# ilyamaclean/microclimf

Hardware: AMD Instinct MI355X
Metric: cell-steps/s (higher is better)
Workload: dtype f64

## Files before the change

microclimf_amd/csrc/mcf_device.hpp:

```cpp
#pragma once
#include <hip/hip_runtime.h>
#include <stdint.h>

#include "mcf_kernels.h"


namespace mcf {

constexpr double kPi = 3.14159265358979323846;
constexpr double kToRad = kPi / 180.0;
constexpr double kSb = 5.67e-8;
constexpr double kThetam = 0.365;
constexpr double kKa = 0.4;
constexpr double kOmdy = (2.0 * kPi) / (24.0 * 3600.0);
constexpr uint64_t kNaRealBits = 0x7FF00000000007A2ULL;

enum : int {
    FL_VALID = 1,
    FL_PAI = 2,
    FL_BELOW = 4,
    FL_XONE = 8,
    FL_XINF = 16,
    FL_XZERO = 32,
    FL_ABOVE1 = 64,
// ... 318 lines not shown
            if (vconst) asm volatile("" : "+s"(t[4]));
            if (vconst) asm volatile("" : "+v"(c5));
            if (vconst || lean_fast) {
                asm volatile("" : "+v"(magic));
                asm volatile("" : "+v"(sh3));
                vfast = true;
            }
        } else {
#pragma unroll
            for (int i = 0; i < 12; ++i) asm volatile("" : "+s"(e[i]));
        }
        if (with_log) {
#pragma unroll
            for (int i = 0; i < 7; ++i)
                if (!logtab) asm volatile("" : "+s"(l[i]));
                else if (i > 0) asm volatile("" : "+s"(g[i]));
            if (logtab && vconst) asm volatile("" : "+v"(g7v));
        }
        if (!vconst) return;
        if (!table) asm volatile("" : "+v"(c11));
        if (with_log && !logtab) { asm volatile("" : "+v"(lg6)); asm volatile("" : "+v"(lg7)); }
    }
};
template <bool BOUNDED, bool SHORT = false>
__device__ __forceinline__ double fexp_tab(double x, const MathK& K) {
    double n, r, p, r2, out;
    int t;
    if (BOUNDED && K.vfast) {
        double y;
        asm("v_fma_f64 %0, %1, %2, %3" : "=v"(y) : "v"(x), "s"(K.t[0]), "v"(K.magic));
        t = __double2loint(y);
        asm("v_add_f64 %0, %1, -%2" : "=v"(n) : "v"(y), "v"(K.magic));
    } else {
        asm("v_mul_f64 %0, %1, %2\n\t"
            "v_rndne_f64 %0, %0"
            : "=v"(n) : "v"(x), "s"(K.t[0]));
        asm("v_cvt_i32_f64 %0, %1" : "=v"(t) : "v"(n));
    }
    if (BOUNDED && SHORT && K.vfast) {
        asm("v_fma_f64 %0, %1, %2, %3" : "=v"(r) : "v"(n), "s"(K.t[4]), "v"(x));
    } else {
        asm("v_fma_f64 %0, %1, %2, %3\n\t"
            "v_fma_f64 %0, %1, %4, %0"
            : "=&v"(r) : "v"(n), "s"(K.t[1]), "v"(x), "s"(K.t[2]));
    }
    double T;
    if (K.vfast) {
        unsigned off;
        asm("v_lshlrev_b32_sdwa %0, %1, %2 dst_sel:DWORD dst_unused:UNUSED_PAD src0_sel:DWORD src1_sel:BYTE_0"
            : "=v"(off) : "v"(K.sh3), "v"(t));
        T = *reinterpret_cast<const double*>(reinterpret_cast<const char*>(K.tab) + off);
    } else {
        T = K.tab[t & 255];
    }
    const int e = t >> 8;
    asm("v_fma_f64 %0, %2, %3, %4\n\t"
        "v_fma_f64 %0, %2, %0, 0.5\n\t"
        "v_mul_f64 %1, %2, %2\n\t"
        "v_fma_f64 %0, %1, %0, %2"
        : "=&v"(p), "=&v"(r2)
        : "v"(r), "s"(K.t[3]), "v"(K.c5));
    asm("v_fma_f64 %0, %1, %2, %1\n\t"
        "v_ldexp_f64 %0, %0, %3"
        : "=&v"(out)
        : "v"(T), "v"(p), "v"(e));
    return out;
}
__device__ __forceinline__ double fexp(double x, const MathK& K);
template <bool F = true>
__device__ __forceinline__ double fexp_b(double x, const MathK& K) {
    if (F && K.table) return fexp_tab<true>(x, K);
    return fexp(x, K);
}
template <bool F = true>
__device__ __forceinline__ double fexp_s(double x, const MathK& K) {
    if (F && K.table) return fexp_tab<true, true>(x, K);
    return fexp(x, K);
}
__device__ __forceinline__ double fexp(double x, const MathK& K) {
    if (K.table) return fexp_tab<false>(x, K);
    double n, r, p, out;
    int t;
    const double c11 = K.c11;
    asm("v_mul_f64 %0, %5, %6\n\t"
        "v_rndne_f64 %0, %0\n\t"
        "v_fma_f64 %1, %0, %7, %5\n\t"
        "v_fma_f64 %1, %0, %8, %1\n\t"
        "v_fma_f64 %2, %1, %9, %10\n\t"
        "v_fma_f64 %2, %1, %2, %11\n\t"
        "v_fma_f64 %2, %1, %2, %12\n\t"
        "v_fma_f64 %2, %1, %2, %13\n\t"
        "v_fma_f64 %2, %1, %2, %14\n\t"
        "v_fma_f64 %2, %1, %2, %15\n\t"
        "v_fma_f64 %2, %1, %2, %16\n\t"
        "v_fma_f64 %2, %1, %2, %17\n\t"
        "v_fma_f64 %2, %1, %2, %18\n\t"
        "v_fma_f64 %2, %1, %2, 1.0\n\t"
        "v_fma_f64 %2, %1, %2, 1.0\n\t"
        "v_cvt_i32_f64 %3, %0\n\t"
        "v_ldexp_f64 %4, %2, %3"
        : "=&v"(n), "=&v"(r), "=&v"(p), "=&v"(t), "=v"(out)
        : "v"(x), "s"(K.e[0]), "s"(K.e[1]), "s"(K.e[2]), "v"(c11), "s"(K.e[3]), "s"(K.e[4]), "s"(K.e[5]), "s"(K.e[6]),
          "s"(K.e[7]), "s"(K.e[8]), "s"(K.e[9]), "s"(K.e[10]), "s"(K.e[11]));
    return out;
}
__device__ __forceinline__ double flog_tab(double x, const MathK& K) {
    const double m = __builtin_amdgcn_frexp_mant(x);
    int e = __builtin_amdgcn_frexp_exp(x);
    const int j = (__double2hiint(m) >> 12) & 255;
    const double2 cl = *reinterpret_cast<const double2*>(K.ltab + 2 * j);
    e -= j < kLogSplit ? 1 : 0;
    const double dk = (double)e;
    double r, q, r2, out;
    asm("v_fma_f64 %0, %4, %5, -1.0\n\t"
        "v_fma_f64 %1, %0, %7, %8\n\t"
        "v_fma_f64 %1, %0, %1, %9\n\t"
        "v_fma_f64 %1, %0, %1, %10\n\t"
        "v_fma_f64 %1, %0, %1, %11\n\t"
        "v_fma_f64 %1, %0, %1, -0.5\n\t"
        "v_mul_f64 %2, %0, %0\n\t"
        "v_fma_f64 %1, %2, %1, %0\n\t"
        "v_fma_f64 %1, %6, %12, %1\n\t"
        "v_fma_f64 %3, %6, %13, %14\n\t"
        "v_add_f64 %3, %3, %1"
        : "=&v"(r), "=&v"(q), "=&v"(r2), "=&v"(out)
        : "v"(m), "v"(cl.x), "v"(dk), "v"(K.g7v), "s"(K.g[1]), "s"(K.g[2]), "s"(K.g[3]), "s"(K.g[4]), "s"(K.g[5]), "s"(K.g[6]),
          "v"(cl.y));
    return out;
}
__device__ __forceinline__ double flog(double x, const MathK& K) {
    if (K.logtab) return flog_tab(x, K);
    double m = __builtin_amdgcn_frexp_mant(x);
    int e = __builtin_amdgcn_frexp_exp(x);
    const int lo = m < 0.70710678118654752440 ? 1 : 0;
    m = __builtin_amdgcn_ldexp(m, lo);
    e -= lo;
    const double f = m - 1.0;
    const double s = fdiv(f, 2.0 + f);
    const double hfsq = 0.5 * f * f;
    const double dk = (double)e;
    const double lg6 = K.lg6, lg7 = K.lg7;
    double z, w, t1, t2, out;
    asm("v_mul_f64 %0, %5, %5\n\t"
        "v_mul_f64 %1, %0, %0\n\t"
        "v_fma_f64 %2, %1, %9, %10\n\t"
        "v_fma_f64 %3, %1, %11, %12\n\t"
        "v_fma_f64 %2, %1, %2, %13\n\t"
        "v_fma_f64 %3, %1, %3, %14\n\t"
        "v_mul_f64 %2, %1, %2\n\t"
        "v_fma_f64 %3, %1, %3, %15\n\t"
        "v_fma_f64 %2, %0, %3, %2\n\t"
        "v_add_f64 %2, %6, %2\n\t"
        "v_mul_f64 %2, %5, %2\n\t"
        "v_fma_f64 %2, %8, %16, %2\n\t"
        "v_add_f64 %2, %6, -%2\n\t"
        "v_add_f64 %2, %2, -%7\n\t"
        "v_fma_f64 %4, %8, %17, -%2"
        : "=&v"(z), "=&v"(w), "=&v"(t1), "=&v"(t2), "=v"(out)
        : "v"(s), "v"(hfsq), "v"(f), "v"(dk), "v"(lg6), "s"(K.l[0]), "v"(lg7), "s"(K.l[1]), "s"(K.l[2]), "s"(K.l[3]),
          "s"(K.l[4]), "s"(K.l[5]), "s"(K.l[6]));
    return out;
}
__device__ __forceinline__ double powxy(double x, double y, const MathK& K) { return fexp(y * flog(x, K), K); }
__device__ __forceinline__ double sq(double x) { return x * x; }
__device__ __forceinline__ double pow4(double x) { double x2 = x * x; return x2 * x2; }

__device__ __forceinline__ void satvap_nd(double tc, double& num, double& den) {
    const bool water = tc > 0;
    const uint64_t m = __builtin_amdgcn_ballot_w64(water);
    if (m == __builtin_amdgcn_ballot_w64(true)) { num = 17.27 * tc; den = tc + 237.3; asm("" : "+v"(num), "+v"(den)); }
    else if (m == 0) { num = 21.875 * tc; den = tc + 265.5; asm("" : "+v"(num), "+v"(den)); }
    else { num = (water ? 17.27 : 21.875) * tc; den = tc + (water ? 237.3 : 265.5); }
}
__device__ __forceinline__ double satvap_arg(double tc) {
    double num, den;
    satvap_nd(tc, num, den);
    return fdiv(num, den);
}
__device__ __forceinline__ void frcp2(double a, double b, double& ra, double& rb) {
    const double r = frcp(a * b);
    ra = r * b;
    rb = r * a;
}
__device__ __forceinline__ void frcp2_m(double a, double b, double& ra, double& rb) {
    const double r = frcp_m(a * b);
    ra = r * b;
    rb = r * a;
}
__device__ __forceinline__ double satvap(double tc, const MathK& K) { return 0.61078 * fexp(satvap_arg(tc), K); }
constexpr double kLnSvp0 = -0x1.f8d9d41e4b1ffp-2;
template <bool F>
__device__ __forceinline__ double satvap_f(double t, const MathK& K) {
    if (F && K.table) {
        double num, den;
        satvap_nd(t, num, den);
        return fexp_s<true>(fma(num, frcp(den), kLnSvp0), K);
    }
    return 0.61078 * fexp_b<F>(satvap_arg(t), K);
}
template <bool F>
__device__ __forceinline__ double satvap_rd(double num, double rden, const MathK& K) {
    if (F && K.table) return fexp_s<true>(fma(num, rden, kLnSvp0), K);
    return 0.61078 * fexp_b<F>(num * rden, K);
}
__device__ __forceinline__ double lw_emit(double tc) { return 0.97 * kSb * pow4(tc + 273.15); }
__device__ __forceinline__ double latent(double tc) {
    return tc >= 0 ? 45068.7 - 42.8428 * tc : 51078.69 - 4.338 * tc - 0.06367 * tc * tc;
}

struct SolPos { double zend, zenr, azid; };

__host__ __device__ inline int julday(int year, int month, int day) {
    double dd = day + 0.5;
    int madj = month + (month < 3) * 12;
    int yadj = year + (month < 3) * -1;
    double j = trunc(365.25 * (yadj + 4716)) + trunc(30.6001 * (madj + 1)) + dd - 1524.5;
    int b = (int)(2 - trunc((double)(yadj / 100)) + trunc(trunc((double)(yadj / 100)) / 4));
    return (int)(j + (j > 2299160) * b);
}

struct SolDate { double sindec, cosdec, eot; };
__device__ inline SolDate sol_date(int year, int month, int day) {
    int jd = julday(year, month, day);
    double m = 6.24004077 + 0.01720197 * (jd - 2451545.0);
    SolDate s;
    s.eot = -7.659 * sin(m) + 9.863 * sin(2 * m + 3.5932);
// ... 205 lines not shown
    __device__ __forceinline__ double operator()(int field) const { return lds_operand(p, field * CPB); }
    __device__ __forceinline__ double hor(int s) const { return lds_operand(p, (CF_COUNT + s) * CPB); }
    __device__ __forceinline__ double wsa(int w) const { return lds_operand(p, (CF_COUNT + 24 + w) * CPB); }
};
struct TimeLds {
    static constexpr bool in_registers = false;
    LdsPtr row;
    __device__ __forceinline__ double operator()(int field) const { return lds_operand(row, field * 24); }
};
struct TimeReg {
    static constexpr bool in_registers = true;
    const TimeVals* t;
    __device__ __forceinline__ double operator()(int field) const { return t->v[field]; }
};

struct Carry {
    double soilm, num0, rden, radCsw, Rddown, Rbdown, X, uf;
};
struct Pass1Out {
    double Tg0, absRnet;
    double uz, Rdup;
};

__device__ __forceinline__ void pin1(double& a) { asm volatile("" : "+v"(a)); }
template <class... A>
__device__ __forceinline__ void pin(A&... a) {
    (pin1(a), ...);
}

#ifndef MCF_CANARY_ALL
#define MCF_CANARY_ALL 0
#endif
struct Canary {
    double c = 0.0;
    __device__ __forceinline__ void watch(double x) { c = fma(0.0, x, c); }
    __device__ __forceinline__ void trip() { c = __builtin_nan(""); }
    __device__ __forceinline__ bool tripped() const { return c != c; }
};
__device__ __forceinline__ void vmin64(double& x, double hi) {
    if (__builtin_constant_p(hi)) {
        if (hi == 1.0) asm("v_min_f64 %0, %0, 1.0" : "+v"(x));
        else asm("v_min_f64 %0, %0, %1" : "+v"(x) : "s"(hi));
    } else asm("v_min_f64 %0, %0, %1" : "+v"(x) : "v"(hi));
}
__device__ __forceinline__ void vmax64(double& x, double lo) {
    if (__builtin_constant_p(lo)) {
        if (lo == 0.0) asm("v_max_f64 %0, %0, 0" : "+v"(x));
        else asm("v_max_f64 %0, %0, %1" : "+v"(x) : "s"(lo));
    } else asm("v_max_f64 %0, %0, %1" : "+v"(x) : "v"(lo));
}
template <bool F>
__device__ __forceinline__ void cap(double& x, double hi, Canary& cn) {
// ... 110 lines not shown
};
struct NoDiag {
    static constexpr bool on = false;
    __device__ __forceinline__ void operator()(int, double) const {}
};
template <int NT>
struct DiagRing {
    static constexpr bool on = true;
    char* day;
    uint64_t sel;
    uint32_t posb;
    __device__ __forceinline__ void operator()(int v, double val) const {
        const unsigned s = (unsigned)(sel >> (4 * v)) & 15u;
        if (s == 15u) return;
        uint32_t pb = posb;
        asm("" : "+v"(pb));
        *(double*)(day + ((size_t)s * (NT * 8)) + pb) = val;
    }
};

template <bool F, bool SS, class CL, class TM, class SL, class DG = NoDiag>
__device__ __forceinline__ void pass1(const CL& C, const TM& T, const SL& S, const Globals& g, int flags, double dTmx,
                                      Carry& cy, Pass1Out& o, const MathK& K, Canary& cn, const DG& dg = NoDiag()) {
    double t_idx = T(TF_IDX), rsw = T(TF_RSW), rdif = T(TF_RDIF);
    pin(t_idx, rsw, rdif);
    const int idx = (int)t_idx;
    constexpr bool soil_shared = SS;
    double soilm, matric;
    if (soil_shared) {
        soilm = S(SD_SOILM);
        matric = S(SD_MATRIC);
    } else {
        double t_soilmp = T(TF_SOILMP), c_smin = C(CF_SMIN), c_invrge = C(CF_INVRGE), c_eta = C(CF_ETA), c_rge = C(CF_RGE);
        pin(t_soilmp, c_smin, c_invrge, c_eta, c_rge);
        soilm = soil_spread<F>(t_soilmp, c_smin, c_invrge, c_eta, c_rge, cn);
        matric = -C(CF_ABSPSIE) * powxy(soilm * C(CF_INVSMAX), -C(CF_SOILB), K);
    }
    cy.soilm = soilm;
    double radGsw = 0.0, radCsw = 0.0, Rbdown = 0.0, Rddown = 0.0, Rdup = 0.0, X = 0.0;
    if constexpr (DG::on) {
        if (!(rsw > 0.0)) {
            double si = T(TF_CZ) * C(CF_CS) + T(TF_SZ) * (C(CF_SSCA) * T(TF_CAZ) + C(CF_SSSA) * T(TF_SAZ));
            if (!g.shadowmask && T(TF_ZEND) > 90.0) si = 0.0;
            flr<F>(si, 0.0, cn);
            if (C.hor(idx & 31) > T(TF_TANSA)) si = 0.0;
            dg(DG_SI, si);
        }
    }
    if (rsw > 0.0) {
        double cz = T(TF_CZ), t_sz = T(TF_SZ), t_caz = T(TF_CAZ), t_saz = T(TF_SAZ), t_tansa = T(TF_TANSA),
               t_zend = T(TF_ZEND);
        double c_cs = C(CF_CS), c_ssca = C(CF_SSCA), c_sssa = C(CF_SSSA), c_hor = C.hor(idx & 31),
               svfa = C(CF_SVFA), gref = C(CF_GREF);
        pin(cz, t_sz, t_caz, t_saz, t_tansa, t_zend, c_cs, c_ssca, c_sssa, c_hor, svfa, gref);
        double si = cz * c_cs + t_sz * (c_ssca * t_caz + c_sssa * t_saz);
        if (!g.shadowmask && t_zend > 90.0) si = 0.0;
        flr<F>(si, 0.0, cn);
        if (c_hor > t_tansa) si = 0.0;
        if constexpr (DG::on) dg(DG_SI, si);
        if (flags & FL_PAI) {
            double t_tan2c = T(TF_TAN2C), t_cosc = T(TF_COSC);
            double c_xx = C(CF_XX), c_kdeninv = C(CF_KDENINV), om = C(CF_OM), gma = C(CF_GMA), agm = C(CF_AGM),
                   u1 = C(CF_U1), u2 = C(CF_U2), c_gma2 = C(CF_GMA2),
                   c_agm2 = C(CF_AGM2), c_jdel = C(CF_JDEL), c_pait = C(CF_PAIT), c_invd2 = C(CF_INVD2), c_gmagref = C(CF_GMAGREF);
            pin(t_tan2c, t_cosc, c_xx, c_kdeninv, om, gma, agm, u1, u2, c_gma2, c_agm2, c_jdel, c_pait, c_invd2, c_gmagref);
            double k = fsqrt(c_xx + t_tan2c) * c_kdeninv;
            if (flags & (FL_XONE | FL_XINF | FL_XZERO))
                k = (flags & FL_XONE) ? T(TF_INV2COSC) : (flags & FL_XINF) ? 1.0 : T(TF_TANC);
            cap<F>(k, 6000.0, cn);
            double rsi = frcp(si);
            double kd = k * t_cosc * rsi;
            double Kc = rsi;
            if (si == 0.0) { kd = 1.0; Kc = 600.0; }
            double sig = kd * kd + c_gma2 - c_agm2;
            double ss = 0.5 * (om * kd + c_jdel);
            double sstr = om * kd - ss;
            double S2 = fexp(-kd * c_pait, K);
            double isig = frcp(sig);
            double p5 = -ss * (agm - kd) - gma * sstr;
            double p5s = p5 * isig;
            double v1 = ss - (p5 * (agm + kd)) * isig;
            double v2 = ss - gma - p5s * (u1 + kd);
            double gS2v2 = S2 * v2;
            double p8 = sstr * (agm + kd) - gma * ss;
            double p8s = -p8 * isig;
            double v3 = (sstr + c_gmagref - p8s * (u2 - kd)) * S2;
            const double dv3 = c_invd2 * v3;
            double c_logclump = C(CF_LOGCLUMP), c_loggi = C(CF_LOGGI), amx = C(CF_AMX), trdn = C(CF_TRDN),
                   trdu = C(CF_TRDU), c_paiaa = C(CF_PAIAA), c_rddng = C(CF_RDDNG), c_albd = C(CF_ALBD), c_rddnz = C(CF_RDDNZ),
                   c_rdupz = C(CF_RDUPZ);
            constexpr bool late_k = TM::in_registers;
            double ka1 = late_k ? 0.0 : C(CF_KA1), ka2 = late_k ? 0.0 : C(CF_KA2), kb1 = late_k ? 0.0 : C(CF_KB1),
                   kb2 = late_k ? 0.0 : C(CF_KB2), kg1 = late_k ? 0.0 : C(CF_KG1), kg2 = late_k ? 0.0 : C(CF_KG2),
                   kz1 = late_k ? 0.0 : C(CF_KZ1), kz2 = late_k ? 0.0 : C(CF_KZ2);
            double Rbeam = T(TF_RBEAM), Rb = T(TF_RB);
            if (late_k) pin(c_logclump, c_loggi, amx, trdn, trdu, c_paiaa, c_rddng, c_albd, c_rddnz, c_rdupz, Rbeam, Rb);
            else pin(c_logclump, c_loggi, amx, trdn, trdu, c_paiaa, c_rddng, c_albd, c_rddnz, c_rdupz, ka1, ka2, kb1, kb2, kg1, kg2, kz1,
                     kz2, Rbeam, Rb);
            double trbn = fexp(Kc * c_logclump, K);
            cap<F>(trbn, 0.999, cn);
            if (!F) flr<F>(trbn, 0.0, cn);
            double trb = fexp(Kc * c_loggi, K);
            cap<F>(trb, 0.999, cn);
            if (!F) flr<F>(trb, 0.0, cn);
            if (late_k) { ka1 = C(CF_KA1); ka2 = C(CF_KA2); }
            double albb = (1.0 - trdn * trbn) * (p5s + (v1 * ka1 + gS2v2 * ka2)) + trdn * trbn * gref;
            if (F) cn.watch(albb);
            cap<F>(albb, amx, cn);
            flr<F>(albb, 0.01, cn);
            if (late_k) { kg1 = C(CF_KG1); kg2 = C(CF_KG2); }
            double Rdbdn_g = (1.0 - trbn) * (p8s * (S2 + kg1) + dv3 * kg2);
            if (F) cn.watch(Rdbdn_g);
            cap<F>(Rdbdn_g, amx, cn);
            flr<F>(Rdbdn_g, 0.0, cn);
            double S2a = fexp(-kd * c_paiaa, K);
            if (late_k) { kb1 = C(CF_KB1); kb2 = C(CF_KB2); }
            double Rdbup_z = (1.0 - trdu * trbn) * (p5s * S2a + (v1 * kb1 + gS2v2 * kb2)) + trdu * trbn * gref;
            cap<F>(Rdbup_z, amx, cn);
            flr<F>(Rdbup_z, 0.0, cn);
            if (late_k) { kz1 = C(CF_KZ1); kz2 = C(CF_KZ2); }
            double Rdbdn_z = (1.0 - trb) * (p8s * (S2a + kz1) + dv3 * kz2);
            cap<F>(Rdbdn_z, amx, cn);
            flr<F>(Rdbdn_z, 0.0, cn);
            double trg = trb + (1 - trb) * S2;
            double Rbc = (trg * si + (1 - trg) * cz) * Rbeam;
            double Rbdn_g = trbn + (1.0 - trbn) * S2;
            if (!F) {
                cap<F>(Rbdn_g, 1.0, cn);
                flr<F>(Rbdn_g, 0.0, cn);
            }
            const double rds = rdif * svfa;
            radGsw = (1.0 - gref) * (c_rddng * rds + Rdbdn_g * Rb + Rbdn_g * Rbeam * si);
            double maxg = (1.0 - gref) * (rds + Rbeam * si);
            cap<F>(radGsw, maxg, cn);
            radCsw = (1.0 - c_albd) * rds + (1.0 - albb) * Rbc;
            Rbdown = (trb + (1.0 - trb) * S2a) * Rbeam;
            Rddown = c_rddnz * rds + Rdbdn_z * Rb;
            Rdup = c_rdupz * rds + Rdbup_z * Rb;
            X = Rddown + Rdup + k * cz * Rbdown;
        } else {
            Rbdown = (rsw - rdif) / cz;
            Rddown = rdif * svfa;
            Rdup = gref * (rdif * svfa + (rsw - rdif));
            radGsw = (1.0 - gref) * (svfa * rdif + si * Rbdown);
            radCsw = radGsw;
        }
    }
    cy.radCsw = radCsw;
    cy.Rddown = Rddown;
    cy.Rbdown = Rbdown;
    cy.X = X;
    o.Rdup = Rdup;
    if constexpr (DG::on) {
        dg(DG_RADGSW, radGsw);
        dg(DG_RADCSW, radCsw);
        const bool lit = rsw > 0.0 && (flags & FL_PAI);
        dg(DG_RADLSW, lit ? C(CF_HOM) * X : 0.0);
        dg(DG_RADLPAR, lit ? C(CF_HOMP) * X : 0.0);
    }
    double c_tsv = C(CF_TSV), c_omtrdif = C(CF_OMTRDIF), ws = C.wsa((idx >> 5) & 7), c_ufc = C(CF_UFC),
           c_uzfac = C(CF_UZFAC), c_ghafac = C(CF_GHAFAC);
    double t_rlw = T(TF_RLW), t_rem = T(TF_REM), u2m = T(TF_U2), t_umu = T(TF_UMU), t_wfac = T(TF_WFAC),
           t_lapk = T(TF_LAPK), t_es = T(TF_ES), t_ea = T(TF_EA), t_ghr = T(TF_GHRRAD), t_de = T(TF_DE),
           tc = T(TF_TC), tdew = T(TF_TDEW);
    pin(c_tsv, c_omtrdif, ws, c_ufc, c_uzfac, c_ghafac, t_rlw, t_rem, u2m, t_umu,
        t_wfac, t_lapk, t_es, t_ea, t_ghr, t_de, tc, tdew);
    const double radGlw = 0.97 * (c_tsv * t_rlw + c_omtrdif * t_rem);
    if constexpr (DG::on) {
        double lwsum = c_tsv * t_rlw + c_omtrdif * t_rem;
        asm volatile("" : "+v"(lwsum));
        const double radGlw_d = 0.97 * lwsum;
        dg(DG_RADGLW, radGlw_d);
        dg(DG_RADCLW, (flags & FL_PAI) ? 0.97 * C(CF_SVFA) * t_rlw : radGlw_d);
        dg(DG_LWOUT, t_rem);
    }
    if (isnan(ws)) ws = 1.0;
    flr<F>(ws, 0.05, cn);
    double uf = u2m * c_ufc * t_umu * ws;
    flr<F>(uf, 0.001, cn);
    double uz = uf * c_uzfac;
    cap<F>(uz, u2m, cn);
    double gHa = uf * c_ghafac;
    flr<F>(gHa, 0.0001, cn);
    cy.uf = uf;
    o.uz = uz;
    if constexpr (DG::on) {
        dg(DG_UF, uf);
        dg(DG_GHA, gHa);
    }
    const double radabs = radGsw + radGlw;
    double surfwet = fexp(matric * t_wfac, K);
    if (!F) cap<F>(surfwet, 1.0, cn);
    const double m = t_lapk * gHa;
    const double num0 = radabs - t_rem - m * (t_es - t_ea) * surfwet;
    const double den = 29.3 * (gHa + t_ghr) + m * t_de;
    cy.num0 = num0;
    const double rden = frcp_m(den);
    cy.rden = rden;
    double Tg0 = pm_temperature_r<F, F && !TM::in_registers>(num0, rden, dTmx, tc, tdew, cn);
    o.Tg0 = Tg0;
    o.absRnet = fabs(radabs - lw_emit(Tg0));
}

struct Stom {
    double gsmax, rsmx, inv02rsmx, gs2;
};
template <bool F>
__device__ __forceinline__ double stomcond(double Rswabs, const Stom& s, const MathK& K, Canary& cn) {
    if (Rswabs <= 0.0) return 0.0;
    double gs = s.gsmax;
    if (Rswabs < s.rsmx) gs = s.gsmax * fexp_s<F>((Rswabs - s.rsmx) * s.inv02rsmx, K);
    cap<F>(gs, s.gs2, cn);
    return gs;
}
// ... 51 lines not shown
    flr<F>(G, -0.6 * Rmx, cn);
    const double Tg = pm_temperature_r<F, F && !TM::in_registers>(cy.num0 - G, cy.rden, dTmx, tc, tdew, cn);
    o.Tg = Tg;
    o.DD = DD;
    if constexpr (DG::on) {
        dg(DG_T0, Tg);
        dg(DG_G, G);
        dg(DG_KDDG, DD);
    }
    if (!above_ground) return;
    constexpr bool lean = TM::in_registers;
    double c_ghafac = C(CF_GHAFAC), c_smin = C(CF_SMIN), c_invrge = C(CF_INVRGE), c_pai = C(CF_PAI),
           c_ksat = C(CF_KSAT), c_psunsat = C(CF_PSUNSAT), c_shadefac = lean ? 0.0 : C(CF_SHADEFAC),
           c_ompc = lean ? 0.0 : C(CF_OMPC), c_svfa = lean ? 0.0 : C(CF_SVFA);
    double rlw = T(TF_RLW), rsw = T(TF_RSW), rdif = T(TF_RDIF), t_idx = T(TF_IDX), lapk = T(TF_LAPK),
           es = T(TF_ES), De = T(TF_DE), rem = T(TF_REM), ghr = T(TF_GHRRAD);
    if (lean) pin(c_ghafac, c_smin, c_invrge, c_pai, c_ksat, c_psunsat);
    else pin(c_ghafac, c_smin, c_invrge, c_pai, c_ksat, c_psunsat, c_shadefac, c_ompc, c_svfa, rlw, rsw, rdif, t_idx,
             lapk, es, De, rem, ghr);
    const double uf = cy.uf;
    double gHa = uf * c_ghafac;
    flr<F>(gHa, 0.0001, cn);
    constexpr bool PAIR = F && !lean;
    const double surfwet = (soilm - c_smin) * c_invrge;
    double esTg = 0.0, dgw = 0.0, gwet = 0.0;
    auto ground_wetness = [&]() {
        double eT = esTg - ea;
        flr<F>(eT, 0.001, cn);
        double plf = 0.8753 - 1.7126 * flog(eT, K);
        dgw = 1.0 + fexp_s<F>(-plf, K);
    };
    if (!PAIR) {
        esTg = satvap_f<F>(Tg, K);
        ground_wetness();
        gwet = frcp(dgw);
        flr<F>(gwet, surfwet, cn);
    }
    const int idx = (int)t_idx;
    double gS = 9999.99;
    Stom st;
    st.gs2 = 0.0;
    bool have_gs2 = false;
    auto load_stom = [&]() {
        if (soil_shared) {
            st.gsmax = C(CF_GSMAX);
            st.rsmx = C(CF_RSMX);
// ... 30 lines not shown
                inv2cosb = 1.0 / (2.0 * cos(zend));
            } else {
                tanb = T(TF_TANB); tan2b = T(TF_TAN2B); inv2cosb = T(TF_INV2COSB);
            }
            kb = fsqrt(C(CF_XX) + tan2b) * C(CF_KDENINV);
            if (flags & (FL_XONE | FL_XINF | FL_XZERO))
                kb = (flags & FL_XONE) ? inv2cosb : (flags & FL_XINF) ? 1.0 : tanb;
            cap<F>(kb, 6000.0, cn);
            P_sun = fdiv_m(1.0 - fexp(-kb * c_pai, K), kb);
        }
        double P_shade = c_pai - P_sun;
        if (lean) { c_shadefac = C(CF_SHADEFAC); c_ompc = C(CF_OMPC); }
        double Rshade_abs = rdif * c_shadefac;
        double Rsun_abs = (rsw - rdif) * kb * (1 - c_ompc) + Rshade_abs;
        double gs_sun = 0.0, gs_shade = 0.0;
        if (!(Rsun_abs <= 0.0) || !(Rshade_abs <= 0.0)) {
            load_stom();
            gs_sun = stomcond<F>(Rsun_abs, st, K, cn);
            gs_shade = stomcond<F>(Rshade_abs, st, K, cn);
        }
        gS = gs_sun * P_sun + gs_shade * P_shade;
    }
    double gV = 0.0;
    if (PAIR) {
        double nTg, dTg, rTg, rG;
        satvap_nd(Tg, nTg, dTg);
        frcp2(dTg, gHa + gS, rTg, rG);
        esTg = satvap_rd<F>(nTg, rTg, K);
        if (gS > 0.0) gV = (gHa * gS) * rG;
        ground_wetness();
    } else if (gS > 0.0) gV = fdiv_m(gHa * gS, gHa + gS);
    if (lean) c_svfa = C(CF_SVFA);
    const double Rabs = cy.radCsw + 0.97 * c_svfa * rlw;
    const double mC = lapk * gV;
    const double esw = (es - ea) * surfwet;
    const double numC = Rabs - rem - mC * esw - G, denC = 29.3 * (gHa + ghr) + mC * De;
    double Tcan;
    if (PAIR) {
        double rC;
        frcp2_m(dgw, denC, gwet, rC);
        flr<F>(gwet, surfwet, cn);
        Tcan = pm_temperature_r<F, F && !lean>(numC, rC, dTmx, tc, tdew, cn);
    } else {
        Tcan = pm_temperature<F, F && !lean>(numC, denC, dTmx, tc, tdew, cn);
    }
    double esTcan, muR = 0.0;
    if (PAIR) {
        double nTc, dTc, rTc;
        satvap_nd(Tcan, nTc, dTc);
        if (flags & FL_BELOW) frcp2(dTc, C(CF_A2H) * uf, rTc, muR);
        else rTc = frcp(dTc);
        esTcan = satvap_rd<F>(nTc, rTc, K);
    } else {
        esTcan = satvap_f<F>(Tcan, K);
    }
    midway();
    double ez;
    if (!(flags & FL_BELOW)) {
        double w = C(CF_OML1);
        bool prof = (flags & FL_ABOVE1) != 0;
        o.Tz = prof ? tc + (Tcan - tc) * w : Tcan;
        ez = prof ? ea + (esTcan - ea) * surfwet * w : ea + (esTcan - ea) * surfwet;
        o.tleaf = Tcan;
        o.lwup = lw_emit(Tcan);
        o.lwdn = rlw;
    } else {
        double c_uzfac = C(CF_UZFAC), emg = C(CF_EMG), ema = C(CF_EMA), invleafd = C(CF_INVLEAFD),
               c_hom = C(CF_HOM), c_homp = C(CF_HOMP), t_u2 = T(TF_U2);
        pin(c_uzfac, emg, ema, invleafd, c_hom, c_homp, t_u2);
        double uz = uf * c_uzfac;
        cap<F>(uz, t_u2, cn);
        const double lwcan = lw_emit(Tcan), lwgro = lw_emit(Tg);
        const double lwup = emg * lwgro + (1 - emg) * lwcan;
        const double lwdn = ema * rlw + (1 - ema) * lwcan;
        const double lwabs = 0.97 * 0.5 * (lwup + lwdn);
        const bool lit = F || (rsw > 0.0 && (flags & FL_PAI));
        const double leafabs = (lit ? c_hom * cy.X : 0.0) + lwabs;
        double gh = (0.135 * 1.4) * fsqrt_m(uz * invleafd);
        const double RnetL = leafabs - lwcan;
        bool floors_idle = false;
        {
            const double tq = gh * (1.0 / 0.0463), tq2 = tq * tq;
            const bool clear = gh >= 0.0500001 && tq2 * tq2 * tq >= (fabs(RnetL) * invleafd) * 1.000001;
            floors_idle = __builtin_amdgcn_ballot_w64(!clear) == 0;
        }
        double a02 = 0.0;
        if (!floors_idle) {
            a02 = mincond_a02<F>(RnetL, invleafd, K, cn);
            double gmin = mincond_gmin<F>(g.hf0p, a02, cn);
            flr<F>(gh, gmin, cn);
        }
        double gVl = gh;
        if (flags & FL_STOM) {
            gVl = 0.0;
            const double PARabs = lit ? c_homp * cy.X : 0.0;
            double gs = 0.0;
            if (PARabs > 0.0) {
                if (!have_gs2) load_stom();
// ... 70 lines not shown
        }
        const double HL = 29.3 * gh * (tleaf - tc);
        const double LL = mL * (esTl - ea) * surfwet;
        const double cp43 = 29.3 * 43.0;
        {
            double Flux = HC * omem, SH = Th * cp43, SG = Tg * cp43;
            double mxnear = fabs(tleaf - Th) * cp43;
            double SC = SH + Flux * rKc;
            double farg = (Kg * SG + Kh * SH + Kc * SC) * invK;
            double near = nf * (HL * lden);
            near_field_limit<F>(near, mxnear);
            o.Tz = (near + farg) * (1.0 / cp43);
        }
        {
            double Flux = LC * omem, SH = eh * mu, SG = esTg * gwet * mu;
            double mxnear = fabs(esTl - eh) * mu;
            double SC = SH + Flux * rKc;
            double farg = (Kg * SG + Kh * SH + Kc * SC) * invK;
            double near = nf * (LL * lden);
            near_field_limit<F>(near, mxnear);
            ez = (near + farg) * invmu;
        }
    }
    double rh;
    if (F) {
        rh = (ez * (100.0 / 0.61078)) * fexp_s<true>(-satvap_arg(o.Tz), K);
    } else {
        rh = fdiv(ez, satvap(o.Tz, K)) * 100.0;
    }
    if (F) cn.watch(rh);
    cap<F>(rh, 100.0, cn);
    o.rh = rh;
    double tmx = o.tleaf;
    flr<F>(tmx, tc, cn);
    flr<F>(tmx, Tg, cn);
    flr<F>(tmx, Tcan, cn);
    double tmn = o.tleaf;
    cap<F>(tmn, tc, cn);
    cap<F>(tmn, Tg, cn);
    cap<F>(tmn, Tcan, cn);
    cap<F>(o.Tz, tmx + 2.0, cn);
    flr<F>(o.Tz, tmn - 2.0, cn);
}

}
```

microclimf_amd/csrc/mcf_kernels.hip:

```cpp
#include <hip/hip_runtime.h>
#include <math.h>
#include <stdio.h>
#include <stdint.h>
#include <algorithm>

#include "mcf_device.hpp"
#include "mcf_kernels.h"

#ifndef MCF_WAVES_PER_EU
#define MCF_WAVES_PER_EU 4
#endif
#ifndef MCF_AF_WAVES
#define MCF_AF_WAVES 3
#endif

namespace mcf {

__global__ void k_fill(double* __restrict__ p, int64_t n, double v) {
    int64_t i = (int64_t)blockIdx.x * blockDim.x + threadIdx.x;
    int64_t stride = (int64_t)gridDim.x * blockDim.x;
    for (; i < n; i += stride) p[i] = v;
}

__global__ void k_gather_cells(RingView src, int64_t step0, int64_t nsteps, const int64_t* __restrict__ cells,
// ... 1634 lines not shown
    double a = x[i], b = y ? y[i] : 0.0, r;
    MathK K;
    K.set();
    __shared__ double s_exptab[256];
    K.use_table(s_exptab, (int)threadIdx.x);
    __shared__ __attribute__((aligned(16))) double s_logtab[512];
    K.use_log_table(s_logtab, (int)threadIdx.x, (int)blockDim.x);
    K.pin(true, true);
    __syncthreads();
    switch (kind) {
        case 0: r = fexp(a, K); break;
        case 1: r = flog(a, K); break;
        case 2: r = fdiv(a, b); break;
        case 3: r = fsqrt(a); break;
        case 4: r = frcp(a); break;
        case 5: r = satvap(a, K); break;
        case 7: r = fexp_b<true>(a, K); break;
        case 8: r = satvap_f<true>(a, K); break;
        case 9: r = fexp_s<true>(a, K); break;
        case 10: r = frcp_m(a); break;
        case 11: r = fsqrt_m(a); break;
        case 12: { double ra, rb; frcp2_m(a, b, ra, rb); r = ra + rb; break; }
        case 13: { double ra, rb; frcp2(a, b, ra, rb); r = ra + rb; break; }
        default: r = powxy(a, b, K); break;
    }
    if (live) out[i] = r;
}
void launch_selftest_math(int kind, const double* x, const double* y, double* out, int64_t n, hipStream_t s) {
    if (n <= 0) return;
    hipLaunchKernelGGL(k_selftest_math, dim3((unsigned)((n + 255) / 256)), dim3(256), 0, s, kind, x, y, out, n);
}

__global__ __launch_bounds__(256) void k_pack_transpose(RingView src, int64_t step0, int64_t rows, int64_t cols,
                                                        double scale, int32_t* __restrict__ dst) {
    __shared__ int32_t tile[32][33];
    const int64_t N = rows * cols;
    const int64_t step = step0 + blockIdx.z;
    int32_t* out = dst + (int64_t)blockIdx.z * N;
    const int tx = threadIdx.x & 31, ty = threadIdx.x >> 5;
    const int64_t r0 = (int64_t)blockIdx.x * 32, c0 = (int64_t)blockIdx.y * 32;
#pragma unroll
    for (int j = ty; j < 32; j += 8) {
        const int64_t r = r0 + tx, c = c0 + j;
        int32_t v = INT32_MIN;
        if (r < rows && c < cols) {
            const double x = rint(src.at(r + rows * c, step) * scale);
// ... 336 lines not shown
```

Baseline: 31.46 billion.

## Split table exp/log into issue and finish phases to hide LDS latency

Splits the LDS-table-based exp and log routines into an issue phase, which computes the index and starts the table load, and a finish phase that evaluates the polynomial. In pass1 and the canopy pass, several exp/log calls are issued early and finished later, with independent arithmetic placed in between to hide LDS load latency. Volatile LDS address-space loads plus register pins keep the compiler from sinking the loads back to their use. The cost is more live VGPRs across the overlap window, which may lower occupancy. Self-test cases for the new paths are added.

```diff
diff --git a/microclimf_amd/csrc/mcf_device.hpp b/microclimf_amd/csrc/mcf_device.hpp
--- a/microclimf_amd/csrc/mcf_device.hpp
+++ b/microclimf_amd/csrc/mcf_device.hpp
@@ -364,9 +364,20 @@
         if (with_log && !logtab) { asm volatile("" : "+v"(lg6)); asm volatile("" : "+v"(lg7)); }
     }
 };
-template <bool BOUNDED, bool SHORT = false>
-__device__ __forceinline__ double fexp_tab(double x, const MathK& K) {
-    double n, r, p, r2, out;
+__device__ __forceinline__ void pin1(double& a) { asm volatile("" : "+v"(a)); }
+template <class... A>
+__device__ __forceinline__ void pin(A&... a) {
+    (pin1(a), ...);
+}
+
+struct ExpPending {
+    double r;
+    int e;
+    double T;
+};
+template <bool BOUNDED, bool SHORT = false, bool HELD = true>
+__device__ __forceinline__ ExpPending fexp_tab_issue(double x, const MathK& K) {
+    double n, r;
     int t;
     if (BOUNDED && K.vfast) {
         double y;
@@ -386,27 +397,42 @@
             "v_fma_f64 %0, %1, %4, %0"
             : "=&v"(r) : "v"(n), "s"(K.t[1]), "v"(x), "s"(K.t[2]));
     }
-    double T;
+    typedef const volatile __attribute__((address_space(3))) char* LdsBytes;
+    typedef const volatile __attribute__((address_space(3))) double* LdsDouble;
+    ExpPending q;
     if (K.vfast) {
         unsigned off;
         asm("v_lshlrev_b32_sdwa %0, %1, %2 dst_sel:DWORD dst_unused:UNUSED_PAD src0_sel:DWORD src1_sel:BYTE_0"
             : "=v"(off) : "v"(K.sh3), "v"(t));
-        T = *reinterpret_cast<const double*>(reinterpret_cast<const char*>(K.tab) + off);
+        if (HELD) q.T = *(LdsDouble)((LdsBytes)K.tab + off);
+        else q.T = *reinterpret_cast<const double*>(reinterpret_cast<const char*>(K.tab) + off);
     } else {
-        T = K.tab[t & 255];
-    }
-    const int e = t >> 8;
+        if (HELD) q.T = ((LdsDouble)K.tab)[t & 255];
+        else q.T = K.tab[t & 255];
+    }
+    q.r = r;
+    q.e = t >> 8;
+    return q;
+}
+template <bool HELD = true>
+__device__ __forceinline__ double fexp_tab_finish(const ExpPending& q, const MathK& K) {
+    double p, r2, out, T = q.T;
     asm("v_fma_f64 %0, %2, %3, %4\n\t"
         "v_fma_f64 %0, %2, %0, 0.5\n\t"
         "v_mul_f64 %1, %2, %2\n\t"
         "v_fma_f64 %0, %1, %0, %2"
         : "=&v"(p), "=&v"(r2)
-        : "v"(r), "s"(K.t[3]), "v"(K.c5));
+        : "v"(q.r), "s"(K.t[3]), "v"(K.c5));
+    if (HELD) pin1(T);
     asm("v_fma_f64 %0, %1, %2, %1\n\t"
         "v_ldexp_f64 %0, %0, %3"
         : "=&v"(out)
-        : "v"(T), "v"(p), "v"(e));
+        : "v"(T), "v"(p), "v"(q.e));
     return out;
+}
+template <bool BOUNDED, bool SHORT = false>
+__device__ __forceinline__ double fexp_tab(double x, const MathK& K) {
+    return fexp_tab_finish<false>(fexp_tab_issue<BOUNDED, SHORT, false>(x, K), K);
 }
 __device__ __forceinline__ double fexp(double x, const MathK& K);
 template <bool F = true>
@@ -446,13 +472,35 @@
           "s"(K.e[7]), "s"(K.e[8]), "s"(K.e[9]), "s"(K.e[10]), "s"(K.e[11]));
     return out;
 }
-__device__ __forceinline__ double flog_tab(double x, const MathK& K) {
-    const double m = __builtin_amdgcn_frexp_mant(x);
-    int e = __builtin_amdgcn_frexp_exp(x);
-    const int j = (__double2hiint(m) >> 12) & 255;
-    const double2 cl = *reinterpret_cast<const double2*>(K.ltab + 2 * j);
-    e -= j < kLogSplit ? 1 : 0;
+struct LogPending {
+    double m;
+    int e, j;
+    double c, l;
+};
+template <bool HELD = true>
+__device__ __forceinline__ LogPending flog_tab_issue(double x, const MathK& K) {
+    LogPending q;
+    q.m = __builtin_amdgcn_frexp_mant(x);
+    q.e = __builtin_amdgcn_frexp_exp(x);
+    q.j = (__double2hiint(q.m) >> 12) & 255;
+    if (HELD) {
+        typedef double __attribute__((ext_vector_type(2))) LdsEntry;
+        const LdsEntry cl = *(const volatile __attribute__((address_space(3))) LdsEntry*)(K.ltab + 2 * q.j);
+        q.c = cl.x;
+        q.l = cl.y;
+    } else {
+        const double2 cl = *reinterpret_cast<const double2*>(K.ltab + 2 * q.j);
+        q.c = cl.x;
+        q.l = cl.y;
+    }
+    return q;
+}
+template <bool HELD = true>
+__device__ __forceinline__ double flog_tab_finish(const LogPending& p, const MathK& K) {
+    const int e = p.e - (p.j < kLogSplit ? 1 : 0);
     const double dk = (double)e;
+    double c = p.c, l = p.l;
+    if (HELD) pin(c, l);
     double r, q, r2, out;
     asm("v_fma_f64 %0, %4, %5, -1.0\n\t"
         "v_fma_f64 %1, %0, %7, %8\n\t"
@@ -466,10 +514,11 @@
         "v_fma_f64 %3, %6, %13, %14\n\t"
         "v_add_f64 %3, %3, %1"
         : "=&v"(r), "=&v"(q), "=&v"(r2), "=&v"(out)
-        : "v"(m), "v"(cl.x), "v"(dk), "v"(K.g7v), "s"(K.g[1]), "s"(K.g[2]), "s"(K.g[3]), "s"(K.g[4]), "s"(K.g[5]), "s"(K.g[6]),
-          "v"(cl.y));
+        : "v"(p.m), "v"(c), "v"(dk), "v"(K.g7v), "s"(K.g[1]), "s"(K.g[2]), "s"(K.g[3]), "s"(K.g[4]), "s"(K.g[5]), "s"(K.g[6]),
+          "v"(l));
     return out;
 }
+__device__ __forceinline__ double flog_tab(double x, const MathK& K) { return flog_tab_finish<false>(flog_tab_issue<false>(x, K), K); }
 __device__ __forceinline__ double flog(double x, const MathK& K) {
     if (K.logtab) return flog_tab(x, K);
     double m = __builtin_amdgcn_frexp_mant(x);
@@ -504,6 +553,42 @@
     return out;
 }
 __device__ __forceinline__ double powxy(double x, double y, const MathK& K) { return fexp(y * flog(x, K), K); }
+struct ExpLater {
+    ExpPending q = {0.0, 0, 0.0};
+    double v = 0.0;
+};
+struct LogLater {
+    LogPending q = {0.0, 0, 0, 0.0, 0.0};
+    double v = 0.0;
+};
+__device__ __forceinline__ ExpLater fexp_issue(double x, const MathK& K) {
+    ExpLater o;
+    if (K.table) o.q = fexp_tab_issue<false>(x, K);
+    else o.v = fexp(x, K);
+    return o;
+}
+template <bool F = true>
+__device__ __forceinline__ ExpLater fexp_b_issue(double x, const MathK& K) {
+    ExpLater o;
+    if (F && K.table) o.q = fexp_tab_issue<true>(x, K);
+    else o = fexp_issue(x, K);
+    return o;
+}
+template <bool F = true>
+__device__ __forceinline__ ExpLater fexp_s_issue(double x, const MathK& K) {
+    ExpLater o;
+    if (F && K.table) o.q = fexp_tab_issue<true, true>(x, K);
+    else o = fexp_issue(x, K);
+    return o;
+}
+__device__ __forceinline__ double fexp_finish(const ExpLater& o, const MathK& K) { return K.table ? fexp_tab_finish(o.q, K) : o.v; }
+__device__ __forceinline__ LogLater flog_issue(double x, const MathK& K) {
+    LogLater o;
+    if (K.logtab) o.q = flog_tab_issue(x, K);
+    else o.v = flog(x, K);
+    return o;
+}
+__device__ __forceinline__ double flog_finish(const LogLater& o, const MathK& K) { return K.logtab ? flog_tab_finish(o.q, K) : o.v; }
 __device__ __forceinline__ double sq(double x) { return x * x; }
 __device__ __forceinline__ double pow4(double x) { double x2 = x * x; return x2 * x2; }
 
@@ -544,6 +629,16 @@
 __device__ __forceinline__ double satvap_rd(double num, double rden, const MathK& K) {
     if (F && K.table) return fexp_s<true>(fma(num, rden, kLnSvp0), K);
     return 0.61078 * fexp_b<F>(num * rden, K);
+}
+template <bool F>
+__device__ __forceinline__ ExpLater satvap_rd_issue(double num, double rden, const MathK& K) {
+    if (F && K.table) return fexp_s_issue<true>(fma(num, rden, kLnSvp0), K);
+    return fexp_b_issue<F>(num * rden, K);
+}
+template <bool F>
+__device__ __forceinline__ double satvap_finish(const ExpLater& o, const MathK& K) {
+    if (F && K.table) return fexp_finish(o, K);
+    return 0.61078 * fexp_finish(o, K);
 }
 __device__ __forceinline__ double lw_emit(double tc) { return 0.97 * kSb * pow4(tc + 273.15); }
 __device__ __forceinline__ double latent(double tc) {
@@ -795,12 +890,6 @@
     double uz, Rdup;
 };
 
-__device__ __forceinline__ void pin1(double& a) { asm volatile("" : "+v"(a)); }
-template <class... A>
-__device__ __forceinline__ void pin(A&... a) {
-    (pin1(a), ...);
-}
-
 #ifndef MCF_CANARY_ALL
 #define MCF_CANARY_ALL 0
 #endif
@@ -957,8 +1046,11 @@
 template <bool F, bool SS, class CL, class TM, class SL, class DG = NoDiag>
 __device__ __forceinline__ void pass1(const CL& C, const TM& T, const SL& S, const Globals& g, int flags, double dTmx,
                                       Carry& cy, Pass1Out& o, const MathK& K, Canary& cn, const DG& dg = NoDiag()) {
-    double t_idx = T(TF_IDX), rsw = T(TF_RSW), rdif = T(TF_RDIF);
+    constexpr bool EARLY = F && !TM::in_registers;
+    constexpr bool E_SW = EARLY, E_A = EARLY, E_B = EARLY;
+    double t_idx = T(TF_IDX), rsw = T(TF_RSW), rdif = T(TF_RDIF), t_wfac = E_SW ? T(TF_WFAC) : 0.0;
     pin(t_idx, rsw, rdif);
+    if (E_SW) pin1(t_wfac);
     const int idx = (int)t_idx;
     constexpr bool soil_shared = SS;
     double soilm, matric;
@@ -972,6 +1064,7 @@
         matric = -C(CF_ABSPSIE) * powxy(soilm * C(CF_INVSMAX), -C(CF_SOILB), K);
     }
     cy.soilm = soilm;
+    const double surfwet_arg = E_SW ? matric * t_wfac : 0.0;
     double radGsw = 0.0, radCsw = 0.0, Rbdown = 0.0, Rddown = 0.0, Rdup = 0.0, X = 0.0;
     if constexpr (DG::on) {
         if (!(rsw > 0.0)) {
@@ -994,11 +1087,12 @@
         if (c_hor > t_tansa) si = 0.0;
         if constexpr (DG::on) dg(DG_SI, si);
         if (flags & FL_PAI) {
-            double t_tan2c = T(TF_TAN2C), t_cosc = T(TF_COSC);
+            double t_tan2c = T(TF_TAN2C), t_cosc = T(TF_COSC), c_logclump = E_A ? C(CF_LOGCLUMP) : 0.0;
             double c_xx = C(CF_XX), c_kdeninv = C(CF_KDENINV), om = C(CF_OM), gma = C(CF_GMA), agm = C(CF_AGM),
                    u1 = C(CF_U1), u2 = C(CF_U2), c_gma2 = C(CF_GMA2),
                    c_agm2 = C(CF_AGM2), c_jdel = C(CF_JDEL), c_pait = C(CF_PAIT), c_invd2 = C(CF_INVD2), c_gmagref = C(CF_GMAGREF);
             pin(t_tan2c, t_cosc, c_xx, c_kdeninv, om, gma, agm, u1, u2, c_gma2, c_agm2, c_jdel, c_pait, c_invd2, c_gmagref);
+            if (E_A) pin1(c_logclump);
             double k = fsqrt(c_xx + t_tan2c) * c_kdeninv;
             if (flags & (FL_XONE | FL_XINF | FL_XZERO))
                 k = (flags & FL_XONE) ? T(TF_INV2COSC) : (flags & FL_XINF) ? 1.0 : T(TF_TANC);
@@ -1010,18 +1104,25 @@
             double sig = kd * kd + c_gma2 - c_agm2;
             double ss = 0.5 * (om * kd + c_jdel);
             double sstr = om * kd - ss;
-            double S2 = fexp(-kd * c_pait, K);
+            ExpLater S2_p, trbn_p, trb_p, S2a_p;
+            double S2 = 0.0;
+            if (E_A) {
+                S2_p = fexp_issue(-kd * c_pait, K);
+                trbn_p = fexp_issue(Kc * c_logclump, K);
+            } else S2 = fexp(-kd * c_pait, K);
             double isig = frcp(sig);
             double p5 = -ss * (agm - kd) - gma * sstr;
             double p5s = p5 * isig;
             double v1 = ss - (p5 * (agm + kd)) * isig;
             double v2 = ss - gma - p5s * (u1 + kd);
+            if (E_A) S2 = fexp_finish(S2_p, K);
             double gS2v2 = S2 * v2;
             double p8 = sstr * (agm + kd) - gma * ss;
             double p8s = -p8 * isig;
             double v3 = (sstr + c_gmagref - p8s * (u2 - kd)) * S2;
             const double dv3 = c_invd2 * v3;
-            double c_logclump = C(CF_LOGCLUMP), c_loggi = C(CF_LOGGI), amx = C(CF_AMX), trdn = C(CF_TRDN),
+            if (!E_A) c_logclump = C(CF_LOGCLUMP);
+            double c_loggi = C(CF_LOGGI), amx = C(CF_AMX), trdn = C(CF_TRDN),
                    trdu = C(CF_TRDU), c_paiaa = C(CF_PAIAA), c_rddng = C(CF_RDDNG), c_albd = C(CF_ALBD), c_rddnz = C(CF_RDDNZ),
                    c_rdupz = C(CF_RDUPZ);
             constexpr bool late_k = TM::in_registers;
@@ -1030,14 +1131,22 @@
                    kz1 = late_k ? 0.0 : C(CF_KZ1), kz2 = late_k ? 0.0 : C(CF_KZ2);
             double Rbeam = T(TF_RBEAM), Rb = T(TF_RB);
             if (late_k) pin(c_logclump, c_loggi, amx, trdn, trdu, c_paiaa, c_rddng, c_albd, c_rddnz, c_rdupz, Rbeam, Rb);
-            else pin(c_logclump, c_loggi, amx, trdn, trdu, c_paiaa, c_rddng, c_albd, c_rddnz, c_rdupz, ka1, ka2, kb1, kb2, kg1, kg2, kz1,
+            else pin(c_loggi, amx, trdn, trdu, c_paiaa, c_rddng, c_albd, c_rddnz, c_rdupz, ka1, ka2, kb1, kb2, kg1, kg2, kz1,
                      kz2, Rbeam, Rb);
-            double trbn = fexp(Kc * c_logclump, K);
+            if (!late_k && !E_A) pin1(c_logclump);
+            double trbn = E_A ? fexp_finish(trbn_p, K) : fexp(Kc * c_logclump, K);
             cap<F>(trbn, 0.999, cn);
             if (!F) flr<F>(trbn, 0.0, cn);
-            double trb = fexp(Kc * c_loggi, K);
-            cap<F>(trb, 0.999, cn);
-            if (!F) flr<F>(trb, 0.0, cn);
+            if (E_B) {
+                trb_p = fexp_issue(Kc * c_loggi, K);
+                S2a_p = fexp_issue(-kd * c_paiaa, K);
+            }
+            double trb = 0.0;
+            if (!E_B) {
+                trb = fexp(Kc * c_loggi, K);
+                cap<F>(trb, 0.999, cn);
+                if (!F) flr<F>(trb, 0.0, cn);
+            }
             if (late_k) { ka1 = C(CF_KA1); ka2 = C(CF_KA2); }
             double albb = (1.0 - trdn * trbn) * (p5s + (v1 * ka1 + gS2v2 * ka2)) + trdn * trbn * gref;
             if (F) cn.watch(albb);
@@ -1048,12 +1157,17 @@
             if (F) cn.watch(Rdbdn_g);
             cap<F>(Rdbdn_g, amx, cn);
             flr<F>(Rdbdn_g, 0.0, cn);
-            double S2a = fexp(-kd * c_paiaa, K);
+            double S2a = E_B ? fexp_finish(S2a_p, K) : fexp(-kd * c_paiaa, K);
             if (late_k) { kb1 = C(CF_KB1); kb2 = C(CF_KB2); }
             double Rdbup_z = (1.0 - trdu * trbn) * (p5s * S2a + (v1 * kb1 + gS2v2 * kb2)) + trdu * trbn * gref;
             cap<F>(Rdbup_z, amx, cn);
             flr<F>(Rdbup_z, 0.0, cn);
             if (late_k) { kz1 = C(CF_KZ1); kz2 = C(CF_KZ2); }
+            if (E_B) {
+                trb = fexp_finish(trb_p, K);
+                cap<F>(trb, 0.999, cn);
+                if (!F) flr<F>(trb, 0.0, cn);
+            }
             double Rdbdn_z = (1.0 - trb) * (p8s * (S2a + kz1) + dv3 * kz2);
             cap<F>(Rdbdn_z, amx, cn);
             flr<F>(Rdbdn_z, 0.0, cn);
@@ -1093,13 +1207,17 @@
         dg(DG_RADLSW, lit ? C(CF_HOM) * X : 0.0);
         dg(DG_RADLPAR, lit ? C(CF_HOMP) * X : 0.0);
     }
+    ExpLater surfwet_p;
+    if (E_SW) surfwet_p = fexp_issue(surfwet_arg, K);
     double c_tsv = C(CF_TSV), c_omtrdif = C(CF_OMTRDIF), ws = C.wsa((idx >> 5) & 7), c_ufc = C(CF_UFC),
            c_uzfac = C(CF_UZFAC), c_ghafac = C(CF_GHAFAC);
-    double t_rlw = T(TF_RLW), t_rem = T(TF_REM), u2m = T(TF_U2), t_umu = T(TF_UMU), t_wfac = T(TF_WFAC),
+    if (!E_SW) t_wfac = T(TF_WFAC);
+    double t_rlw = T(TF_RLW), t_rem = T(TF_REM), u2m = T(TF_U2), t_umu = T(TF_UMU),
            t_lapk = T(TF_LAPK), t_es = T(TF_ES), t_ea = T(TF_EA), t_ghr = T(TF_GHRRAD), t_de = T(TF_DE),
            tc = T(TF_TC), tdew = T(TF_TDEW);
     pin(c_tsv, c_omtrdif, ws, c_ufc, c_uzfac, c_ghafac, t_rlw, t_rem, u2m, t_umu,
-        t_wfac, t_lapk, t_es, t_ea, t_ghr, t_de, tc, tdew);
+        t_lapk, t_es, t_ea, t_ghr, t_de, tc, tdew);
+    if (!E_SW) pin1(t_wfac);
     const double radGlw = 0.97 * (c_tsv * t_rlw + c_omtrdif * t_rem);
     if constexpr (DG::on) {
         double lwsum = c_tsv * t_rlw + c_omtrdif * t_rem;
@@ -1124,7 +1242,7 @@
         dg(DG_GHA, gHa);
     }
     const double radabs = radGsw + radGlw;
-    double surfwet = fexp(matric * t_wfac, K);
+    double surfwet = E_SW ? fexp_finish(surfwet_p, K) : fexp(matric * t_wfac, K);
     if (!F) cap<F>(surfwet, 1.0, cn);
     const double m = t_lapk * gHa;
     const double num0 = radabs - t_rem - m * (t_es - t_ea) * surfwet;
@@ -1222,6 +1340,7 @@
     double gHa = uf * c_ghafac;
     flr<F>(gHa, 0.0001, cn);
     constexpr bool PAIR = F && !lean;
+    constexpr bool P_CH = PAIR, P_TC = PAIR, P_RH = F;
     const double surfwet = (soilm - c_smin) * c_invrge;
     double esTg = 0.0, dgw = 0.0, gwet = 0.0;
     auto ground_wetness = [&]() {
@@ -1298,19 +1417,32 @@
         gS = gs_sun * P_sun + gs_shade * P_shade;
     }
     double gV = 0.0;
+    ExpLater esTg_p;
+    LogLater eT_p;
     if (PAIR) {
         double nTg, dTg, rTg, rG;
         satvap_nd(Tg, nTg, dTg);
         frcp2(dTg, gHa + gS, rTg, rG);
-        esTg = satvap_rd<F>(nTg, rTg, K);
+        if (P_CH) esTg_p = satvap_rd_issue<F>(nTg, rTg, K);
+        else esTg = satvap_rd<F>(nTg, rTg, K);
         if (gS > 0.0) gV = (gHa * gS) * rG;
-        ground_wetness();
+        if (!P_CH) ground_wetness();
     } else if (gS > 0.0) gV = fdiv_m(gHa * gS, gHa + gS);
     if (lean) c_svfa = C(CF_SVFA);
     const double Rabs = cy.radCsw + 0.97 * c_svfa * rlw;
     const double mC = lapk * gV;
     const double esw = (es - ea) * surfwet;
+    if (P_CH) {
+        esTg = satvap_finish<F>(esTg_p, K);
+        double eT = esTg - ea;
+        flr<F>(eT, 0.001, cn);
+        eT_p = flog_issue(eT, K);
+    }
     const double numC = Rabs - rem - mC * esw - G, denC = 29.3 * (gHa + ghr) + mC * De;
+    if (P_CH) {
+        double plf = 0.8753 - 1.7126 * flog_finish(eT_p, K);
+        dgw = 1.0 + fexp_s<F>(-plf, K);
+    }
     double Tcan;
     if (PAIR) {
         double rC;
@@ -1320,13 +1452,15 @@
     } else {
         Tcan = pm_temperature<F, F && !lean>(numC, denC, dTmx, tc, tdew, cn);
     }
-    double esTcan, muR = 0.0;
+    double esTcan = 0.0, muR = 0.0;
+    ExpLater esTcan_p;
     if (PAIR) {
         double nTc, dTc, rTc;
         satvap_nd(Tcan, nTc, dTc);
         if (flags & FL_BELOW) frcp2(dTc, C(CF_A2H) * uf, rTc, muR);
         else rTc = frcp(dTc);
-        esTcan = satvap_rd<F>(nTc, rTc, K);
+        if (P_TC) esTcan_p = satvap_rd_issue<F>(nTc, rTc, K);
+        else esTcan = satvap_rd<F>(nTc, rTc, K);
     } else {
         esTcan = satvap_f<F>(Tcan, K);
     }
@@ -1336,6 +1470,7 @@
         double w = C(CF_OML1);
         bool prof = (flags & FL_ABOVE1) != 0;
         o.Tz = prof ? tc + (Tcan - tc) * w : Tcan;
+        if (P_TC) esTcan = satvap_finish<F>(esTcan_p, K);
         ez = prof ? ea + (esTcan - ea) * surfwet * w : ea + (esTcan - ea) * surfwet;
         o.tleaf = Tcan;
         o.lwup = lw_emit(Tcan);
@@ -1350,6 +1485,7 @@
         const double lwup = emg * lwgro + (1 - emg) * lwcan;
         const double lwdn = ema * rlw + (1 - ema) * lwcan;
         const double lwabs = 0.97 * 0.5 * (lwup + lwdn);
+        if (P_TC) esTcan = satvap_finish<F>(esTcan_p, K);
         const bool lit = F || (rsw > 0.0 && (flags & FL_PAI));
         const double leafabs = (lit ? c_hom * cy.X : 0.0) + lwabs;
         double gh = (0.135 * 1.4) * fsqrt_m(uz * invleafd);
@@ -1466,15 +1602,8 @@
             ez = (near + farg) * invmu;
         }
     }
-    double rh;
-    if (F) {
-        rh = (ez * (100.0 / 0.61078)) * fexp_s<true>(-satvap_arg(o.Tz), K);
-    } else {
-        rh = fdiv(ez, satvap(o.Tz, K)) * 100.0;
-    }
-    if (F) cn.watch(rh);
-    cap<F>(rh, 100.0, cn);
-    o.rh = rh;
+    ExpLater rh_p;
+    if (P_RH) rh_p = fexp_s_issue<true>(-satvap_arg(o.Tz), K);
     double tmx = o.tleaf;
     flr<F>(tmx, tc, cn);
     flr<F>(tmx, Tg, cn);
@@ -1483,6 +1612,15 @@
     cap<F>(tmn, tc, cn);
     cap<F>(tmn, Tg, cn);
     cap<F>(tmn, Tcan, cn);
+    double rh;
+    if (F) {
+        rh = (ez * (100.0 / 0.61078)) * (P_RH ? fexp_finish(rh_p, K) : fexp_s<true>(-satvap_arg(o.Tz), K));
+    } else {
+        rh = fdiv(ez, satvap(o.Tz, K)) * 100.0;
+    }
+    if (F) cn.watch(rh);
+    cap<F>(rh, 100.0, cn);
+    o.rh = rh;
     cap<F>(o.Tz, tmx + 2.0, cn);
     flr<F>(o.Tz, tmn - 2.0, cn);
 }
diff --git a/microclimf_amd/csrc/mcf_kernels.hip b/microclimf_amd/csrc/mcf_kernels.hip
--- a/microclimf_amd/csrc/mcf_kernels.hip
+++ b/microclimf_amd/csrc/mcf_kernels.hip
@@ -1680,6 +1680,18 @@
         case 11: r = fsqrt_m(a); break;
         case 12: { double ra, rb; frcp2_m(a, b, ra, rb); r = ra + rb; break; }
         case 13: { double ra, rb; frcp2(a, b, ra, rb); r = ra + rb; break; }
+        case 14: { const ExpLater p = fexp_issue(a, K); r = fexp_finish(p, K); break; }
+        case 15: { const ExpLater p = fexp_b_issue<true>(a, K); r = fexp_finish(p, K); break; }
+        case 16: { const ExpLater p = fexp_s_issue<true>(a, K); r = fexp_finish(p, K); break; }
+        case 17: { const LogLater p = flog_issue(a, K); r = flog_finish(p, K); break; }
+        case 18: case 19: case 20: {
+            const ExpLater p0 = fexp_issue(a, K);
+            const ExpLater p1 = fexp_b_issue<true>(b, K);
+            const LogLater p2 = flog_issue(a, K);
+            const double r2 = flog_finish(p2, K), r1 = fexp_finish(p1, K), r0 = fexp_finish(p0, K);
+            r = kind == 18 ? r0 : kind == 19 ? r1 : r2;
+            break;
+        }
         default: r = powxy(a, b, K); break;
     }
     if (live) out[i] = r;
```

Result: no change. 31.45 billion (median of 4 runs) (-0.0%).
